# CESNET/GPUJPEG

Measured on NVIDIA H100. Metric: Mpix/s encode+decode 8k RGB q75, higher is better.
Workload: dtype f32+i32 (u8 in, i16 coefficients)

## Files before the change

### gpujpeg_b200/csrc/gj_dct.cu

```cuda
#include <cuda_runtime.h>
#include <stdint.h>
#include <stdlib.h>
#include <string.h>

#include <tuple>
#include <type_traits>

#include "gj_device.cuh"
#include "gj_internal.h"
#include "gj_launch.cuh"

namespace {

constexpr int TB = 64;
constexpr int NT = 192;
constexpr int STRIP_PX = TB * 8;
constexpr int GROUPS = 8 * (STRIP_PX / 4);
constexpr int BLK_F = 68;
constexpr int K1_SMEM = 3 * TB * BLK_F * 4;
constexpr int K1_OUT_STRIDE = 9;
constexpr int K4_PLANE = 8 * STRIP_PX;

struct FdctParams {
    float fwd_zz[2][64];
};
struct IdctParams {
    uint16_t q_zz[GJ_MAX_COMP][64];
};

__device__ __forceinline__ uint32_t pack4_sat_u8(int p0, int p1, int p2, int p3)
{
    uint32_t hi, d;
    asm("cvt.pack.sat.u8.s32.b32 %0, %1, %2, %3;" : "=r"(hi) : "r"(p3), "r"(p2), "r"(0));
    asm("cvt.pack.sat.u8.s32.b32 %0, %1, %2, %3;" : "=r"(d) : "r"(p1), "r"(p0), "r"(hi));
    return d;
}

__device__ __forceinline__ uint64_t quantise_pack(const float (&v)[64], const float* __restrict__ tab, uint32_t (&packed)[32])
{
    uint32_t mlo = 0, mhi = 0;
#pragma unroll
    for ( int k = 0; k < 64; k += 2 ) {
        const uint32_t b0 = gj_quant_bits(v[gj_zz2nat(k)], tab[k]);
        const uint32_t b1 = gj_quant_bits(v[gj_zz2nat(k + 1)], tab[k + 1]);
        packed[k >> 1] = __byte_perm(b0, b1, 0x5410);
        if ( k < 32 ) {
            if ( b0 != GJ_QUANT_ZERO ) mlo |= 1u << (k & 31);
            if ( b1 != GJ_QUANT_ZERO ) mlo |= 1u << ((k + 1) & 31);
        }
        else {
            if ( b0 != GJ_QUANT_ZERO ) mhi |= 1u << (k & 31);
            if ( b1 != GJ_QUANT_ZERO ) mhi |= 1u << ((k + 1) & 31);
        }
    }
    return (uint64_t)mhi << 32 | mlo;
}
__device__ __forceinline__ void quantise_store(const float (&v)[64], const float* __restrict__ tab, int16_t* __restrict__ coef_blk,
                                               uint64_t* __restrict__ nz)
{
    uint32_t packed[32];
    *nz = quantise_pack(v, tab, packed);
    uint4* dst = reinterpret_cast<uint4*>(coef_blk);
#pragma unroll
    for ( int i = 0; i < 8; i++ )
        dst[i] = make_uint4(packed[4 * i], packed[4 * i + 1], packed[4 * i + 2], packed[4 * i + 3]);
}


template <int VEC>
__global__ void __launch_bounds__(NT)
k_fdct_rgb444(const uint8_t* __restrict__ raw, int width, int height, size_t pitch, int16_t* __restrict__ coef,
              uint64_t* __restrict__ nzmask, int bcx, int nblk, const __grid_constant__ FdctParams prm)
{
    gj_pdl_wait();
    extern __shared__ __align__(16) uint8_t smem[];
    float* s_pl = reinterpret_cast<float*>(smem);

    const int bx0 = blockIdx.x * TB;
    const int by = blockIdx.y;
    const int x0 = bx0 * 8;
    const int vw = min(STRIP_PX, width - x0);
    const int vh = min(8, height - by * 8);
    const uint8_t* src = raw + (size_t)by * 8 * pitch + (size_t)x0 * 3;

    constexpr int ITERS = (GROUPS + NT - 1) / NT;
    uint32_t w0[ITERS], w1[ITERS], w2[ITERS];
#pragma unroll
    for ( int it = 0; it < ITERS; it++ ) {
        const int g = threadIdx.x + it * NT;
        const int row = g >> 7, gx = g & 127, px0 = gx * 4;
        w0[it] = w1[it] = w2[it] = 0u;
        if ( g < GROUPS && row < vh && px0 < vw ) {
            const uint8_t* p = src + (size_t)row * pitch + gx * 12;
            if ( VEC == 4 && px0 + 4 <= vw ) {
                const uint32_t* w = reinterpret_cast<const uint32_t*>(p);
                w0[it] = __ldg(w);
                w1[it] = __ldg(w + 1);
                w2[it] = __ldg(w + 2);
            }
            else {
                const int nb = min(12, (vw - px0) * 3);
                uint32_t b[12];
#pragma unroll
                for ( int i = 0; i < 12; i++ )
                    b[i] = i < nb ? (uint32_t)__ldg(p + i) : 0u;
                w0[it] = b[0] | b[1] << 8 | b[2] << 16 | b[3] << 24;
                w1[it] = b[4] | b[5] << 8 | b[6] << 16 | b[7] << 24;
                w2[it] = b[8] | b[9] << 8 | b[10] << 16 | b[11] << 24;
            }
        }
    }
#pragma unroll
    for ( int it = 0; it < ITERS; it++ ) {
        const int g = threadIdx.x + it * NT;
        if ( g >= GROUPS ) break;
        const int row = g >> 7, gx = g & 127, px0 = gx * 4;
        float4 y4 = make_float4(0.f, 0.f, 0.f, 0.f), cb4 = y4, cr4 = y4;
        if ( row < vh && px0 < vw ) {
            const uint32_t a0 = w0[it], a1 = w1[it], a2 = w2[it];
            gj_rgb_to_ycbcr_m(gj_byte_as_magic(a0, 0), gj_byte_as_magic(a0, 1), gj_byte_as_magic(a0, 2), y4.x, cb4.x, cr4.x);
            gj_rgb_to_ycbcr_m(gj_byte_as_magic(a0, 3), gj_byte_as_magic(a1, 0), gj_byte_as_magic(a1, 1), y4.y, cb4.y, cr4.y);
            gj_rgb_to_ycbcr_m(gj_byte_as_magic(a1, 2), gj_byte_as_magic(a1, 3), gj_byte_as_magic(a2, 0), y4.z, cb4.z, cr4.z);
            gj_rgb_to_ycbcr_m(gj_byte_as_magic(a2, 1), gj_byte_as_magic(a2, 2), gj_byte_as_magic(a2, 3), y4.w, cb4.w, cr4.w);
            if ( px0 + 4 > vw ) {
                if ( px0 + 1 >= vw ) { y4.y = cb4.y = cr4.y = 0.f; }
                if ( px0 + 2 >= vw ) { y4.z = cb4.z = cr4.z = 0.f; }
                if ( px0 + 3 >= vw ) { y4.w = cb4.w = cr4.w = 0.f; }
            }
        }
        const int off = (gx >> 1) * BLK_F + row * 8 + (gx & 1) * 4;
        *reinterpret_cast<float4*>(s_pl + off) = y4;
        *reinterpret_cast<float4*>(s_pl + TB * BLK_F + off) = cb4;
        *reinterpret_cast<float4*>(s_pl + 2 * TB * BLK_F + off) = cr4;
    }
    __syncthreads();

    const int comp = threadIdx.x >> 6;
    const int b = threadIdx.x & 63;
    const bool active = bx0 + b < bcx;
    float v[64];
    {
        const float4* in = reinterpret_cast<const float4*>(s_pl + (comp * TB + b) * BLK_F);
#pragma unroll
        for ( int i = 0; i < 16; i++ ) {
            const float4 t = in[i];
            v[4 * i] = t.x; v[4 * i + 1] = t.y; v[4 * i + 2] = t.z; v[4 * i + 3] = t.w;
        }
    }
    __syncthreads();
    gj_fdct_block(v);
    uint4* const s_out = reinterpret_cast<uint4*>(smem);
    {
        uint32_t packed[32];
        const uint64_t nz = quantise_pack(v, prm.fwd_zz[comp == 0 ? 0 : 1], packed);
        const size_t bi = (size_t)comp * nblk + (size_t)by * bcx + bx0 + b;
        if ( active ) nzmask[bi] = nz;
#pragma unroll
        for ( int i = 0; i < 8; i++ )
            s_out[threadIdx.x * K1_OUT_STRIDE + i] = make_uint4(packed[4 * i], packed[4 * i + 1], packed[4 * i + 2], packed[4 * i + 3]);
    }
    __syncthreads();
#pragma unroll
    for ( int k = 0; k < 8; k++ ) {
        const int q = threadIdx.x + k * NT;
        const int slot = q >> 3, part = q & 7;
        const int c2 = slot >> 6, b2 = slot & 63;
        if ( bx0 + b2 < bcx ) {
            const size_t bi = (size_t)c2 * nblk + (size_t)by * bcx + bx0 + b2;
            reinterpret_cast<uint4*>(coef + bi * 64)[part] = s_out[slot * K1_OUT_STRIDE + part];
        }
    }
}

constexpr int K1T_RAW = 8 * STRIP_PX * 3;
constexpr int K1T_SMEM = K1_SMEM + K1T_RAW + 16;

__device__ __forceinline__ uint32_t smem_u32(const void* p) { return (uint32_t)__cvta_generic_to_shared(p); }
__device__ __forceinline__ void mbar_init(uint32_t bar, uint32_t count)
{
    asm volatile("mbarrier.init.shared::cta.b64 [%0], %1;" ::"r"(bar), "r"(count));
}
__device__ __forceinline__ void mbar_expect_tx(uint32_t bar, uint32_t bytes)
{
    asm volatile("mbarrier.arrive.expect_tx.shared::cta.b64 _, [%0], %1;" ::"r"(bar), "r"(bytes) : "memory");
}
__device__ __forceinline__ void mbar_wait(uint32_t bar, uint32_t parity)
{
    asm volatile(
        "{\n"
        ".reg .pred p;\n"
        "WAIT_%=:\n"
        "mbarrier.try_wait.parity.shared::cta.b64 p, [%0], %1;\n"
        "@p bra DONE_%=;\n"
        "bra WAIT_%=;\n"
        "DONE_%=:\n"
        "}\n" ::"r"(bar),
        "r"(parity)
        : "memory");
}
__device__ __forceinline__ void bulk_g2s(uint32_t dst, const void* src, uint32_t bytes, uint32_t bar)
{
    asm volatile("cp.async.bulk.shared::cluster.global.mbarrier::complete_tx::bytes [%0], [%1], %2, [%3];" ::"r"(dst), "l"(src),
// ... 53 lines not shown
            *reinterpret_cast<float4*>(s_pl + off) = y4;
            *reinterpret_cast<float4*>(s_pl + TB * BLK_F + off) = cb4;
            *reinterpret_cast<float4*>(s_pl + 2 * TB * BLK_F + off) = cr4;
        }
        __syncthreads();
        if ( threadIdx.x == 0 && strip + (int)gridDim.x < n_strips ) {
            asm volatile("fence.proxy.async.shared::cta;" ::: "memory");
            request(strip + gridDim.x);
        }

        const int comp = threadIdx.x >> 6;
        const int b = threadIdx.x & 63;
        if ( bx0 + b < bcx ) {
            float v[64];
            const float4* in = reinterpret_cast<const float4*>(s_pl + (comp * TB + b) * BLK_F);
#pragma unroll
            for ( int i = 0; i < 16; i++ ) {
                const float4 t = in[i];
                v[4 * i] = t.x; v[4 * i + 1] = t.y; v[4 * i + 2] = t.z; v[4 * i + 3] = t.w;
            }
            gj_fdct_block(v);
            const size_t bi = (size_t)comp * nblk + (size_t)by * bcx + bx0 + b;
            quantise_store(v, prm.fwd_zz[comp == 0 ? 0 : 1], coef + bi * 64, nzmask + bi);
        }
        __syncthreads();
    }
}

struct SsGrid {
    int bcx[3], bcy[3], blk_off[3];
};

template <int HS, int VS, int VEC>
__global__ void __launch_bounds__(TB * VS + 2 * TB / HS)
k_fdct_rgb_ss(const uint8_t* __restrict__ raw, int width, int height, size_t pitch, int16_t* __restrict__ coef,
              uint64_t* __restrict__ nzmask, const __grid_constant__ SsGrid grid, const __grid_constant__ FdctParams prm)
{
    gj_pdl_wait();
    constexpr int NTS = TB * VS + 2 * TB / HS;
    constexpr int CB = TB / HS;
    constexpr int ITERS = (GROUPS + NTS - 1) / NTS;
    extern __shared__ __align__(16) uint8_t smem[];
    float* s_y = reinterpret_cast<float*>(smem);
    float* s_c = s_y + VS * TB * BLK_F;

    const int bx0 = blockIdx.x * TB;
    const int x0 = bx0 * 8;
    const int y0 = blockIdx.y * 8 * VS;
    const int vw = min(STRIP_PX, width - x0);
    const uint8_t* src = raw + (size_t)y0 * pitch + (size_t)x0 * 3;

#pragma unroll
    for ( int half = 0; half < VS; half++ ) {
        const int vh = min(8, height - y0 - half * 8);
        uint32_t w0[ITERS], w1[ITERS], w2[ITERS];
#pragma unroll
        for ( int it = 0; it < ITERS; it++ ) {
            const int g = threadIdx.x + it * NTS;
            const int row = g >> 7, gx = g & 127, px0 = gx * 4;
            w0[it] = w1[it] = w2[it] = 0u;
            if ( g < GROUPS && row < vh && px0 < vw ) {
                const uint8_t* p = src + (size_t)(half * 8 + row) * pitch + gx * 12;
                if ( VEC == 4 && px0 + 4 <= vw ) {
                    const uint32_t* w = reinterpret_cast<const uint32_t*>(p);
                    w0[it] = __ldg(w);
                    w1[it] = __ldg(w + 1);
                    w2[it] = __ldg(w + 2);
                }
                else {
                    const int nb = min(12, (vw - px0) * 3);
                    uint32_t b[12];
#pragma unroll
                    for ( int i = 0; i < 12; i++ )
                        b[i] = i < nb ? (uint32_t)__ldg(p + i) : 0u;
                    w0[it] = b[0] | b[1] << 8 | b[2] << 16 | b[3] << 24;
                    w1[it] = b[4] | b[5] << 8 | b[6] << 16 | b[7] << 24;
                    w2[it] = b[8] | b[9] << 8 | b[10] << 16 | b[11] << 24;
                }
            }
        }
#pragma unroll
        for ( int it = 0; it < ITERS; it++ ) {
            const int g = threadIdx.x + it * NTS;
            if ( g >= GROUPS ) break;
            const int row = g >> 7, gx = g & 127, px0 = gx * 4;
            float4 y4 = make_float4(0.f, 0.f, 0.f, 0.f), cb4 = y4, cr4 = y4;
            if ( row < vh && px0 < vw ) {
                const uint32_t a0 = w0[it], a1 = w1[it], a2 = w2[it];
                gj_rgb_to_ycbcr_m(gj_byte_as_magic(a0, 0), gj_byte_as_magic(a0, 1), gj_byte_as_magic(a0, 2), y4.x, cb4.x, cr4.x);
                gj_rgb_to_ycbcr_m(gj_byte_as_magic(a0, 3), gj_byte_as_magic(a1, 0), gj_byte_as_magic(a1, 1), y4.y, cb4.y, cr4.y);
                gj_rgb_to_ycbcr_m(gj_byte_as_magic(a1, 2), gj_byte_as_magic(a1, 3), gj_byte_as_magic(a2, 0), y4.z, cb4.z, cr4.z);
                gj_rgb_to_ycbcr_m(gj_byte_as_magic(a2, 1), gj_byte_as_magic(a2, 2), gj_byte_as_magic(a2, 3), y4.w, cb4.w, cr4.w);
                if ( px0 + 4 > vw ) {
                    if ( px0 + 1 >= vw ) { y4.y = cb4.y = cr4.y = 0.f; }
                    if ( px0 + 2 >= vw ) { y4.z = cb4.z = cr4.z = 0.f; }
                    if ( px0 + 3 >= vw ) { y4.w = cb4.w = cr4.w = 0.f; }
                }
            }
            *reinterpret_cast<float4*>(s_y + (half * TB + (gx >> 1)) * BLK_F + row * 8 + (gx & 1) * 4) = y4;
            const int srow = half * 8 + row;
            if ( VS == 1 || (srow & 1) == 0 ) {
                const int crow = srow / VS;
                if ( HS == 1 ) {
                    const int off = (gx >> 1) * BLK_F + crow * 8 + (gx & 1) * 4;
                    *reinterpret_cast<float4*>(s_c + off) = cb4;
                    *reinterpret_cast<float4*>(s_c + CB * BLK_F + off) = cr4;
                }
                else {
                    const int off = (gx >> 2) * BLK_F + crow * 8 + (gx & 3) * 2;
                    *reinterpret_cast<float2*>(s_c + off) = make_float2(cb4.x, cb4.z);
                    *reinterpret_cast<float2*>(s_c + CB * BLK_F + off) = make_float2(cr4.x, cr4.z);
                }
            }
        }
    }
    __syncthreads();

    auto locate = [&](int t, int& comp, int& bx, int& by) {
        if ( t < TB * VS ) {
            comp = 0;
            bx = bx0 + (t & (TB - 1));
            by = blockIdx.y * VS + t / TB;
        }
        else {
            const int u = t - TB * VS;
            comp = 1 + u / CB;
            bx = bx0 / HS + u % CB;
            by = blockIdx.y;
        }
        return bx < grid.bcx[comp] && by < grid.bcy[comp];
    };
    int comp, bx, by;
    const bool active = locate(threadIdx.x, comp, bx, by);
    float v[64];
    {
        const float4* in = reinterpret_cast<const float4*>(s_y + threadIdx.x * BLK_F);
#pragma unroll
        for ( int i = 0; i < 16; i++ ) {
            const float4 t = in[i];
            v[4 * i] = t.x; v[4 * i + 1] = t.y; v[4 * i + 2] = t.z; v[4 * i + 3] = t.w;
        }
    }
    __syncthreads();
    gj_fdct_block(v);
    uint4* const s_out = reinterpret_cast<uint4*>(smem);
    {
        uint32_t packed[32];
        const uint64_t nz = quantise_pack(v, prm.fwd_zz[comp == 0 ? 0 : 1], packed);
        if ( active ) nzmask[(size_t)grid.blk_off[comp] + (size_t)by * grid.bcx[comp] + bx] = nz;
#pragma unroll
        for ( int i = 0; i < 8; i++ )
            s_out[threadIdx.x * K1_OUT_STRIDE + i] = make_uint4(packed[4 * i], packed[4 * i + 1], packed[4 * i + 2], packed[4 * i + 3]);
    }
    __syncthreads();
#pragma unroll
    for ( int k = 0; k < 8; k++ ) {
        const int q = threadIdx.x + k * NTS;
        const int slot = q >> 3, part = q & 7;
        int c2, bx2, by2;
        if ( locate(slot, c2, bx2, by2) ) {
            const size_t bi = (size_t)grid.blk_off[c2] + (size_t)by2 * grid.bcx[c2] + bx2;
            reinterpret_cast<uint4*>(coef + bi * 64)[part] = s_out[slot * K1_OUT_STRIDE + part];
        }
    }
}

struct LjGrid {
    int bcx[3], bcy[3], blk_off[3];
    int wib[3], hib[3];
};
struct LjParams {
    uint32_t recip[2][64];
    uint16_t q[2][64];
};

template <int HS, int VS, int NC>
struct LjShape {
    static constexpr int NTS = TB * VS + (NC == 3 ? 2 * TB / HS : 0);
    static constexpr int CB = TB / HS;
    static constexpr int PLANE = 8 * VS * STRIP_PX;
    static constexpr int OUT = NTS * K1_OUT_STRIDE * 16;
    static constexpr int SMEM = (NC * PLANE > OUT ? NC * PLANE : OUT) + NTS * 4;
};

template <int N>
__device__ __forceinline__ void lj_row(const uint8_t* __restrict__ row, int x, int vw, int (&out)[N])
{
    if ( x + N <= vw ) {
        const uint32_t* w = reinterpret_cast<const uint32_t*>(row + x);
#pragma unroll
        for ( int i = 0; i < N / 4; i++ ) {
            const uint32_t v = w[i];
#pragma unroll
            for ( int j = 0; j < 4; j++ )
                out[4 * i + j] = (int)((v >> (8 * j)) & 255u);
// ... 1208 lines not shown
```

### gpujpeg_b200/csrc/gj_decoder.c

```c
#include <stdlib.h>
#include <string.h>

#include "gj_internal.h"

#define GJ_MK_OTHER_CAP 256
#define GJ_CTA_BYTES0 (64 * 1024)
#define GJ_MK_WORDS (8 + 4 * GJ_MK_OTHER_CAP)

#define GJ_STRIPES 8
#define GJ_STRIPE_MIN_BYTES ((size_t)8 << 20)

struct gpujpeg_decoder {
    gj_stream_t stream;
    gj_stream_t copy_stream;
    void* ev_stripe[GJ_STRIPES]; void* ev_done;
    int stripes;
    size_t stripe_min_bytes;
    int k3_parts;
    int device;
    int verbose, perf_stats;
    struct gpujpeg_parameters param;
    struct gpujpeg_image_parameters param_image;
    struct gj_geometry geo;
    int initialised;
// ... 1547 lines not shown

GPUJPEG_API int gpujpegx_decoder_subsequence_rounds(struct gpujpeg_decoder* d)
{
    if ( !d || !d->last_valid || !d->used_subsequences ) return -1;
    return gj_subseq_rounds(d->d_ss_scratch, d->stream);
}

GPUJPEG_API int gpujpegx_decoder_run_resident(struct gpujpeg_decoder* d, uint8_t* d_out, int stage_mask)
{
    if ( !d || !d->last_valid ) return -1;
    if ( d->last_progressive ) {
        static const int comp_tq[GJ_MAX_COMP] = {0, 1, 2, 3};
        if ( (stage_mask & 4) &&
             gj_launch_marker_scan(d->d_file, d->last_ecs_begin, d->last_args.file_size, d->d_cta, d->d_list_pos, d->d_list_code,
                                   d->d_list_cpos, d->last_list_cap, d->d_clean, d->d_mk, d->d_mk + 8, GJ_MK_OTHER_CAP, d->stream) )
            return -1;
        if ( (stage_mask & 1) && gj_launch_progressive_decode(&d->last_prog, d->stream) ) return -1;
        if ( (stage_mask & 2) && launch_k4(d, comp_tq, d_out ? d_out : d->d_raw, 0, d->k4.mcu_rows) ) return -1;
        return 0;
    }
    if ( (stage_mask & 4) && !d->used_segment_info &&
         gj_launch_marker_scan(d->d_file, d->last_ecs_begin, d->last_args.file_size, d->d_cta, d->d_list_pos, d->d_list_code,
                               d->d_list_cpos, d->last_list_cap, d->d_clean, d->d_mk, d->d_mk + 8, GJ_MK_OTHER_CAP, d->stream) )
        return -1;
    if ( (stage_mask & 1) && d->crop && gj_cuda_memset_async(d->d_cext, 0, d->geo.coef_count / 64, d->stream) ) return -1;
    if ( (stage_mask & 1) && gj_launch_huffman_decode(&d->last_args, d->stream) ) return -1;
    if ( (stage_mask & 2) && launch_k4(d, d->last_tq, d_out ? d_out : d->d_raw, 0, d->k4.mcu_rows) ) return -1;
    return 0;
}

GPUJPEG_API int gpujpegx_decoder_get_coefficients(struct gpujpeg_decoder* d, int16_t* out, size_t count)
{
    if ( !d || !d->initialised || !d->last_valid || count != d->geo.coef_count ) return -1;
    if ( gj_coef_to_host_natural(d->d_coef, d->d_cext, count, out, d->stream) ) return -1;
    return d->k4.dequantize;
}
```

### gpujpeg_b200/csrc/gj_device.cuh

```cuda
#ifndef GJ_DEVICE_CUH
#define GJ_DEVICE_CUH

#include <stdint.h>
#include <math.h>

#include "gj_internal.h"

#if defined(__CUDA_ARCH__)
#define GJ_HD __host__ __device__ __forceinline__
#define GJ_FADD(a, b) __fadd_rn((a), (b))
#define GJ_FSUB(a, b) __fsub_rn((a), (b))
#define GJ_FMUL(a, b) __fmul_rn((a), (b))
#define GJ_FMA(a, b, c) __fmaf_rn((a), (b), (c))
#define GJ_RINT(a) __float2int_rn(a)
#elif defined(__CUDACC__)
#define GJ_HD __host__ __device__ __forceinline__
#define GJ_FADD(a, b) ((a) + (b))
#define GJ_FSUB(a, b) ((a) - (b))
#define GJ_FMUL(a, b) ((a) * (b))
#define GJ_FMA(a, b, c) fmaf((a), (b), (c))
#define GJ_RINT(a) ((int)rintf(a))
#else
#define GJ_HD static inline
#define GJ_FADD(a, b) ((a) + (b))
// ... 1 lines not shown
#define GJ_FMUL(a, b) ((a) * (b))
#define GJ_FMA(a, b, c) fmaf((a), (b), (c))
#define GJ_RINT(a) ((int)rintf(a))
#endif


GJ_HD constexpr int gj_zz2nat(int k)
{
    constexpr int t[64] = {0,  1,  8,  16, 9,  2,  3,  10, 17, 24, 32, 25, 18, 11, 4,  5,  12, 19, 26, 33, 40, 48,
                           41, 34, 27, 20, 13, 6,  7,  14, 21, 28, 35, 42, 49, 56, 57, 50, 43, 36, 29, 22, 15, 23,
                           30, 37, 44, 51, 58, 59, 52, 45, 38, 31, 39, 46, 53, 60, 61, 54, 47, 55, 62, 63};
    return t[k];
}
GJ_HD constexpr int gj_nat2zz(int n)
{
    constexpr int t[64] = {0,  1,  5,  6,  14, 15, 27, 28, 2,  4,  7,  13, 16, 26, 29, 42, 3,  8,  12, 17, 25, 30,
                           41, 43, 9,  11, 18, 24, 31, 40, 44, 53, 10, 19, 23, 32, 39, 45, 52, 54, 20, 22, 33, 38,
                           46, 51, 55, 60, 21, 34, 37, 47, 50, 56, 59, 61, 35, 36, 48, 49, 57, 58, 62, 63};
    return t[n];
}

GJ_HD int gj_coef_src(int k, int transpose, int neg_x, int neg_y, int* negate)
{
    const int n = gj_zz2nat(k), v = n >> 3, u = n & 7;
    const int sv = transpose ? u : v, su = transpose ? v : u;
    *negate = ((neg_x & su) ^ (neg_y & sv)) & 1;
    return gj_nat2zz(sv * 8 + su);
}


GJ_HD int gj_cext_of(int last_zz) { return (last_zz >> 3) + 1; }
GJ_HD bool gj_cext_holds(int ext, int k) { return (k >> 3) < ext; }

#if defined(__CUDACC__)
__device__ __forceinline__ void gj_load_coef_block(const int16_t* __restrict__ blk, int ext, uint32_t (&packed)[32])
{
    const uint4* src = reinterpret_cast<const uint4*>(blk);
#pragma unroll
    for ( int i = 0; i < 8; i++ ) {
        const uint4 t = i < ext ? __ldg(src + i) : make_uint4(0u, 0u, 0u, 0u);
        packed[4 * i] = t.x; packed[4 * i + 1] = t.y; packed[4 * i + 2] = t.z; packed[4 * i + 3] = t.w;
    }
}
#endif


#define GJ_MAGIC23 8388608.0f
#define GJ_MAGIC15 12582912.0f
GJ_HD float gj_byte_as_magic(uint32_t word, int i)
{
#if defined(__CUDA_ARCH__)
    return __uint_as_float(__byte_perm(word, 0x4B000000u, 0x7440 + i));
#else
    union { uint32_t u; float f; } c;
    c.u = 0x4B000000u | ((word >> (8 * i)) & 0xFFu);
    return c.f;
#endif
}
GJ_HD float gj_scale255_m(float cm) { return fmaxf(cm, fmaf(cm, 2.0f, -(GJ_MAGIC23 + 254.0f))) - GJ_MAGIC23; }
GJ_HD float gj_round_clamp255(float acc) { return fminf(acc + GJ_MAGIC15, GJ_MAGIC15 + 255.0f) - GJ_MAGIC15; }
GJ_HD void gj_rgb_to_ycbcr_m(float rm, float gm, float bm, float& y, float& cb, float& cr)
{
    const float r = gj_scale255_m(rm), g = gj_scale255_m(gm), b = gj_scale255_m(bm);
    const float e = 1.0f / 512.0f;
    y = gj_round_clamp255(fmaf(77.0f / 256.0f, r, fmaf(150.0f / 256.0f, g, fmaf(29.0f / 256.0f, b, e))));
    cb = gj_round_clamp255(fmaf(-43.0f / 256.0f, r, fmaf(-85.0f / 256.0f, g, fmaf(128.0f / 256.0f, b, 128.0f + e))));
    cr = gj_round_clamp255(fmaf(128.0f / 256.0f, r, fmaf(-107.0f / 256.0f, g, fmaf(-21.0f / 256.0f, b, 128.0f + e))));
}
GJ_HD void gj_rgb_to_ycbcr(float r, float g, float b, float& y, float& cb, float& cr)
{
    gj_rgb_to_ycbcr_m(r + GJ_MAGIC23, g + GJ_MAGIC23, b + GJ_MAGIC23, y, cb, cr);
}

GJ_HD int gj_clamp8(int v) { return v < 0 ? 0 : (v > 255 ? 255 : v); }
GJ_HD void gj_ycbcr_to_rgb_raw(int Y, int Cb, int Cr, int& r, int& g, int& b)
{
    const int y = Y * 256 + ((Y + 1) & 0x100) + 128;
    const int cb = Cb - 128, cr = Cr - 128;
    r = (y + 359 * cr) >> 8;
    g = (y - 88 * cb - 183 * cr) >> 8;
    b = (y + 454 * cb) >> 8;
}
GJ_HD void gj_ycbcr_to_rgb(int Y, int Cb, int Cr, int& r, int& g, int& b)
{
    gj_ycbcr_to_rgb_raw(Y, Cb, Cr, r, g, b);
    r = gj_clamp8(r);
    g = gj_clamp8(g);
    b = gj_clamp8(b);
}


GJ_HD void gj_fdct1(float& a0, float& a1, float& a2, float& a3, float& a4, float& a5, float& a6, float& a7,
                    const float shift)
{
    const float d0 = GJ_FADD(a0, a7), d1 = GJ_FADD(a1, a6), d2 = GJ_FADD(a2, a5), d3 = GJ_FADD(a3, a4);
    const float d4 = GJ_FSUB(a3, a4), d5 = GJ_FSUB(a2, a5), d6 = GJ_FSUB(a1, a6), d7 = GJ_FSUB(a0, a7);
    const float e0 = GJ_FADD(d0, d3), e1 = GJ_FADD(d1, d2), e2 = GJ_FSUB(d1, d2), e3 = GJ_FSUB(d0, d3);
    const float ed = GJ_FADD(e2, e3);
    const float o0 = GJ_FADD(d4, d5), o1 = GJ_FADD(d5, d6), o2 = GJ_FADD(d6, d7);
    const float od5 = GJ_FMUL(GJ_FSUB(o0, o2), 0.382683433f);
    const float od4 = GJ_FMA(1.306562965f, o2, od5);
    const float od3 = GJ_FMA(-0.707106781f, o1, d7);
    const float od2 = GJ_FMA(0.541196100f, o0, od5);
    const float od1 = GJ_FMA(0.707106781f, o1, d7);
// ... 911 lines not shown
```

### gpujpeg_b200/csrc/gj_encoder.c

```c
#include <assert.h>
#include <stdlib.h>
#include <string.h>

#include "gj_internal.h"

#define GJ_STRIPES 8
#define GJ_STRIPE_MIN_BYTES ((size_t)8 << 20)

struct gpujpeg_encoder {
    gj_stream_t stream;
    int device;
    struct gpujpeg_parameters param;
    struct gpujpeg_image_parameters param_image;
    int initialised;
    struct gj_geometry geo;
    int input_mode;
    uint8_t* d_planes; size_t d_planes_size;
    struct gj_raw_layout raw;
    int quality;
    enum gpujpeg_header_type header_type;
    enum gpujpeg_header_type header_written;
    int flipped;
    int flip_mode;
    unsigned channel_remap;
// ... 1137 lines not shown
    if ( (stage_mask & 1) && launch_k1(e, d_raw) ) return -1;
    if ( (stage_mask & 8) && launch_stats(e) ) return -1;
    if ( (stage_mask & 2) && launch_k2(e) ) return -1;
    return 0;
}

GPUJPEG_API int gpujpegx_encoder_get_symbol_counts(struct gpujpeg_encoder* e, uint64_t out[2][2][256])
{
    if ( !e || !e->initialised || !e->counts_valid || !out ) return -1;
    if ( gj_cuda_memcpy_d2h_async(e->h_counts, e->d_counts, GJ_HUFF_COUNTS_BYTES, e->stream) || gj_cuda_stream_sync(e->stream) )
        return -1;
    memcpy(out, e->h_counts, GJ_HUFF_COUNTS_BYTES);
    return 0;
}

GPUJPEG_API long long gpujpegx_encoder_get_stream(struct gpujpeg_encoder* e, uint8_t* out, size_t capacity)
{
    if ( !e || !e->initialised || e->with_segment_info || !e->d_info_cur ) return -1;
    if ( gj_cuda_memcpy_d2h_async(e->h_info, e->d_info_cur, 32, e->stream) || gj_cuda_stream_sync(e->stream) ) return -1;
    const size_t total = (size_t)e->h_info[0];
    if ( e->h_info[1] || total < e->header_size + 2 || total > e->d_stream_size ) return -1;
    if ( !out ) return (long long)total;
    if ( total > capacity ) return -1;
    if ( gj_cuda_memcpy_d2h_async(out + e->header_size, e->d_stream + e->header_size, total - e->header_size, e->stream) ||
         gj_cuda_stream_sync(e->stream) )
        return -1;
    memcpy(out, e->header, e->header_size);
    return (long long)total;
}

GPUJPEG_API int gpujpegx_encoder_get_coefficients(struct gpujpeg_encoder* e, int16_t* out, size_t count)
{
    if ( !e || !e->initialised || count != e->geo.coef_count ) return -1;
    return gj_coef_to_host_natural(e->d_coef, NULL, count, out, e->stream);
}
```

### gpujpeg_b200/csrc/gj_huffman.cu

```cuda
#include <cuda_runtime.h>
#include <stdint.h>

#include "gj_device.cuh"
#include "gj_internal.h"
#include "gj_launch.cuh"

namespace {

constexpr unsigned FULL = 0xFFFFFFFFu;

__device__ __forceinline__ int warp_incl_scan(int v, int lane)
{
#pragma unroll
    for ( int d = 1; d < 32; d <<= 1 ) {
        const int t = __shfl_up_sync(FULL, v, d);
        if ( lane >= d ) v += t;
    }
    return v;
}

__device__ __forceinline__ int scan_of_segment(const gj_scan_layout& L, int g)
{
    return (g >= L.scan_seg_begin[1]) + (g >= L.scan_seg_begin[2]) + (g >= L.scan_seg_begin[3]);
}
// ... 1293 lines not shown
            uint4* dst = reinterpret_cast<uint4*>(s_cmp);
            for ( uint32_t i = lane; i < (need + 3u) >> 2; i += 32 )
                dst[i] = __ldg(src + i);
        }
        __syncwarp();
        const uint32_t* w = staged ? s_cmp + ((cs >> 2) - wbase) : a.d_clean + (cs >> 2);
        CleanSource c;
        c.n = 0;
        if ( live ) src_init(c, w, w + ((ce >> 2) - (cs >> 2)) + 4, (cs & 3u) * 8u);
        decode_blocks(c);
    }
    else {
        BitSource r;
        r.n = 0;
        if ( live ) src_init(r, file + start, file_end);
        decode_blocks(r);
    }
}

__global__ void __launch_bounds__(256) k_rst_check(const __grid_constant__ gj_huff_dec_args a)
{
    gj_pdl_wait();
    const int g = blockIdx.x * 256 + threadIdx.x;
    if ( g >= a.seg_count ) return;
    const int scan = scan_of_segment(a.lay, g);
    const int s = g - a.lay.scan_seg_begin[scan];
    if ( s > 0 && a.d_list_code[a.first_rank[scan] + (uint32_t)s - 1u] != (uint8_t)(0xD0 + ((s - 1) & 7)) ) atomicExch(a.d_error, 1u);
}

__constant__ uint8_t c_zz2nat[64] = {
    0,  1,  8,  16, 9,  2,  3,  10, 17, 24, 32, 25, 18, 11, 4,  5,  12, 19, 26, 33, 40, 48,
    41, 34, 27, 20, 13, 6,  7,  14, 21, 28, 35, 42, 49, 56, 57, 50, 43, 36, 29, 22, 15, 23,
    30, 37, 44, 51, 58, 59, 52, 45, 38, 31, 39, 46, 53, 60, 61, 54, 47, 55, 62, 63};
__global__ void k_coef_to_natural(const int16_t* __restrict__ in, const uint8_t* __restrict__ cext, int16_t* __restrict__ out,
                                  size_t nblocks)
{
    const size_t i = (size_t)blockIdx.x * blockDim.x + threadIdx.x;
    if ( i >= nblocks * 64 ) return;
    const int k = (int)(i & 63);
    out[(i & ~(size_t)63) + c_zz2nat[k]] = !cext || gj_cext_holds(cext[i >> 6], k) ? in[i] : (int16_t)0;
}

}

static unsigned long long* place_status_of(const struct gj_huff_enc_args* a) { return reinterpret_cast<unsigned long long*>(a->d_seg_off); }

extern "C" int gj_huffman_encode_parts_eligible(const struct gj_huff_enc_args* a)
{
    return a->lay.simple && a->seg_mcu * a->lay.bpm <= HP_MAXBLK;
}

extern "C" int gj_launch_huffman_encode_part(const struct gj_huff_enc_args* a, int first, const int lo[GJ_MAX_COMP],
                                             const int n[GJ_MAX_COMP], gj_stream_t stream)
{
    const int seg_count = a->lay.scan_seg_begin[GJ_MAX_COMP];
    if ( a->seg_mcu * a->lay.bpm > HP_MAXBLK ) return -1;
    if ( first && !a->info_is_zero && cudaMemsetAsync(a->d_info, 0, 32, stream) != cudaSuccess ) return -1;
    SegPick pick;
    pick.total = 0;
    pick.zero_status = first;
    for ( int k = 0; k < GJ_MAX_COMP; k++ ) {
        const bool real = k < a->lay.scan_count;
        pick.n[k] = real ? n[k] : 0;
        pick.lo[k] = real ? a->lay.scan_seg_begin[k] + lo[k] : 0;
        if ( pick.n[k] < 0 || (real && (lo[k] < 0 || pick.lo[k] + pick.n[k] > a->lay.scan_seg_begin[k + 1])) ) return -1;
        pick.total += pick.n[k];
    }
    if ( pick.total == 0 && !first ) return 0;
    const int n_status = (seg_count + CP_SEGS - 1) / CP_SEGS;
    static int attr_done_p[64];
    int dev = 0;
    if ( cudaGetDevice(&dev) != cudaSuccess || dev < 0 || dev >= 64 ) return -1;
    if ( !__atomic_load_n(&attr_done_p[dev], __ATOMIC_ACQUIRE) ) {
// ... 157 lines not shown
        const int cmp_max = (int)(HD_THREADS / 32 * HD_CMP_MAX + 64);
        if ( cudaFuncSetAttribute(k_huff_decode<true, true, false>, cudaFuncAttributeMaxDynamicSharedMemorySize, cmp_max) != cudaSuccess ||
             cudaFuncSetAttribute(k_huff_decode<false, true, false>, cudaFuncAttributeMaxDynamicSharedMemorySize, cmp_max) != cudaSuccess ||
             cudaFuncSetAttribute(k_huff_decode<true, true, true>, cudaFuncAttributeMaxDynamicSharedMemorySize, cmp_max) != cudaSuccess ||
             cudaFuncSetAttribute(k_huff_decode<false, true, true>, cudaFuncAttributeMaxDynamicSharedMemorySize, cmp_max) != cudaSuccess )
            return -1;
        __atomic_store_n(&attr_done[dev], 1, __ATOMIC_RELEASE);
    }
    auto launch = [&](auto kernel) {
        gj_launch_pdl(kernel, dim3(grid), dim3(HD_THREADS), smem, stream, a->d_file, a->d_file + a->file_size, a->d_seg_off,
                      owners, a->seg_mcu, *a, own, a->d_coef, a->d_cext, a->d_tables);
    };
    if ( pick ) {
        if ( own.cmp_words ) {
            if ( a->dequantize ) launch(k_huff_decode<true, true, true>);
            else launch(k_huff_decode<false, true, true>);
        }
        else {
            if ( a->dequantize ) launch(k_huff_decode<true, false, true>);
            else launch(k_huff_decode<false, false, true>);
        }
    }
    else if ( own.cmp_words ) {
        if ( a->dequantize ) launch(k_huff_decode<true, true, false>);
        else launch(k_huff_decode<false, true, false>);
    }
    else {
        if ( a->dequantize ) launch(k_huff_decode<true, false, false>);
        else launch(k_huff_decode<false, false, false>);
    }
    return cudaGetLastError() == cudaSuccess ? 0 : -1;
}

extern "C" int gj_coef_to_host_natural(const int16_t* d_coef, const uint8_t* d_cext, size_t count, int16_t* h_out, gj_stream_t stream)
{
    int16_t* d_tmp = nullptr;
    if ( cudaMalloc(&d_tmp, count * sizeof(int16_t)) != cudaSuccess ) return -1;
    const size_t nblocks = count / 64;
    k_coef_to_natural<<<(unsigned)((count + 255) / 256), 256, 0, stream>>>(d_coef, d_cext, d_tmp, nblocks);
    cudaMemcpyAsync(h_out, d_tmp, count * sizeof(int16_t), cudaMemcpyDeviceToHost, stream);
    const cudaError_t e = cudaStreamSynchronize(stream);
    cudaFree(d_tmp);
    return e == cudaSuccess ? 0 : -1;
}
```

### gpujpeg_b200/csrc/gj_internal.h

```cpp
#ifndef GJ_INTERNAL_H
#define GJ_INTERNAL_H

#include <stddef.h>
#include <stdint.h>
#include <stdio.h>

#include "../../include/gpujpeg_b200.h"

#ifdef __cplusplus
extern "C" {
#endif

#define GJ_MAX_COMP 4
#define GJ_SOS_LEN_1 10

#define GJ_ERR(...) (void)(fprintf(stderr, "[GPUJPEG] [Error] " __VA_ARGS__))
#define GJ_WARN(...) (void)(fprintf(stderr, "[GPUJPEG] [Warning] " __VA_ARGS__))
#define GJ_VERBOSE(v, ...) do { if ( (v) >= GPUJPEG_LL_VERBOSE ) (void)fprintf(stderr, "[GPUJPEG] [Verbose] " __VA_ARGS__); } while ( 0 )
#define GJ_DEBUG(v, ...) do { if ( (v) >= GPUJPEG_LL_DEBUG ) (void)fprintf(stderr, "[GPUJPEG] [Debug] " __VA_ARGS__); } while ( 0 )

extern const uint8_t gj_zigzag_to_natural[64];
extern const uint8_t gj_natural_to_zigzag[64];

struct gj_huff_spec {
// ... 456 lines not shown
    const uint8_t* d_cext;
    int src_blk_off[GJ_MAX_COMP];
    int16_t* d_dst;
    uint64_t* d_nzmask;
    int dst_blk_off[GJ_MAX_COMP];
    int comp_count;
    int dst_blocks;
    int transpose, neg_x, neg_y;
    struct gj_blk_map blk[GJ_MAX_COMP];
    uint32_t* d_range;
};
int gj_launch_coef_transform(const struct gj_coef_transform_args* a, gj_stream_t stream);

struct gj_coef_frame {
    const struct gj_geometry* geo;
    const int16_t* d_coef;
    const uint8_t* d_cext;
    int progressive;
    enum gpujpeg_color_space color_space;
    uint8_t qt[GJ_MAX_COMP][64];
    int tq[GJ_MAX_COMP];
    struct gpujpeg_image_metadata metadata;
    const uint8_t* com;
    size_t com_size;
};
int gj_decoder_decode_coefficients(struct gpujpeg_decoder* d, const uint8_t* image, size_t image_size, struct gj_coef_frame* f);

int gj_encoder_setup_coefficients(struct gpujpeg_encoder* e, const struct gpujpeg_parameters* p, int width, int height,
                                  const uint8_t comp_q[GJ_MAX_COMP][64], const uint8_t comp_tq[GJ_MAX_COMP], const uint8_t* com,
                                  size_t com_size, const struct gpujpeg_image_metadata* metadata, int16_t** d_coef,
                                  uint64_t** d_nzmask, const struct gj_geometry** geo);
int gj_encoder_finish(struct gpujpeg_encoder* e, uint8_t** out, size_t* out_size);

int gj_coef_to_host_natural(const int16_t* d_coef, const uint8_t* d_cext, size_t count, int16_t* h_out, gj_stream_t stream);

int gj_cuda_malloc(void** p, size_t size);
int gj_cuda_free(void* p);
int gj_cuda_malloc_host(void** p, size_t size);
int gj_cuda_free_host(void* p);
int gj_cuda_memcpy_h2d_async(void* dst, const void* src, size_t size, gj_stream_t s);
int gj_cuda_memcpy_d2h_async(void* dst, const void* src, size_t size, gj_stream_t s);
int gj_cuda_memcpy_d2d_async(void* dst, const void* src, size_t size, gj_stream_t s);
int gj_cuda_memset_async(void* dst, int v, size_t size, gj_stream_t s);
int gj_cuda_stream_sync(gj_stream_t s);
int gj_cuda_stream_create(gj_stream_t* s);
int gj_cuda_event_create(void** ev);
void gj_cuda_event_destroy(void* ev);
int gj_cuda_event_record(void* ev, gj_stream_t s);
int gj_cuda_stream_wait_event(gj_stream_t s, void* ev);
void gj_cuda_stream_destroy(gj_stream_t s);
int gj_cuda_enable_peer(int peer);
int gj_cuda_memcpy_peer_async(void* dst, int dst_dev, const void* src, int src_dev, size_t size, gj_stream_t s);
int gj_cuda_pointer_is_device(const void* p);
const char* gj_cuda_last_error(void);
struct gj_timer { void* start; void* stop; int armed; };
int gj_timer_create(struct gj_timer* t);
void gj_timer_destroy(struct gj_timer* t);
void gj_timer_start(struct gj_timer* t, gj_stream_t s);
void gj_timer_stop(struct gj_timer* t, gj_stream_t s);
double gj_timer_ms(struct gj_timer* t);
int gj_cuda_device_count(void);
int gj_cuda_sm_count(void);
int gj_cuda_device_props(int dev, struct gpujpeg_device_info* info);
int gj_cuda_set_device(int dev);
int gj_cuda_get_device(void);
void gj_cuda_device_reset(void);

// ... 5 lines not shown
```

Measured before the change: 58620.

## Store only live coefficient chunks and use dp4a integer color conversion

The forward DCT kernels now write only the 16-byte coefficient chunks up to the last nonzero zigzag position, as derived from the nonzero mask, and skip the trailing zero chunks. The goal is to cut global write traffic. Consumers must then treat the unwritten chunks as zero, so the coefficient export masks them using nzmask. The RGB to YCbCr step is replaced by an integer dp4a/byte-permute version, which may change rounding. The subsampled kernel also gets a minimum-blocks-per-SM launch bound.

After: 60670 (median of 6 runs). +3.5%, better.

```diff
diff --git a/gpujpeg_b200/csrc/gj_dct.cu b/gpujpeg_b200/csrc/gj_dct.cu
--- a/gpujpeg_b200/csrc/gj_dct.cu
+++ b/gpujpeg_b200/csrc/gj_dct.cu
@@ -19,6 +19,7 @@
 constexpr int BLK_F = 68;
 constexpr int K1_SMEM = 3 * TB * BLK_F * 4;
 constexpr int K1_OUT_STRIDE = 9;
+constexpr int k1_ctas_per_sm(int nt) { return 228 * 1024 / (nt * BLK_F * 4 + 1024); }
 constexpr int K4_PLANE = 8 * STRIP_PX;
 
 struct FdctParams {
@@ -64,6 +65,39 @@
 #pragma unroll
     for ( int i = 0; i < 8; i++ )
         dst[i] = make_uint4(packed[4 * i], packed[4 * i + 1], packed[4 * i + 2], packed[4 * i + 3]);
+}
+
+__device__ __forceinline__ void ycc4_clipped(uint32_t w0, uint32_t w1, uint32_t w2, int left, float4& y4, float4& cb4, float4& cr4)
+{
+    float y[4], cb[4], cr[4];
+    gj_rgb4_to_ycbcr(w0, w1, w2, y, cb, cr);
+    y4 = make_float4(y[0], y[1], y[2], y[3]);
+    cb4 = make_float4(cb[0], cb[1], cb[2], cb[3]);
+    cr4 = make_float4(cr[0], cr[1], cr[2], cr[3]);
+    if ( left < 4 ) {
+        if ( left <= 1 ) { y4.y = cb4.y = cr4.y = 0.f; }
+        if ( left <= 2 ) { y4.z = cb4.z = cr4.z = 0.f; }
+        if ( left <= 3 ) { y4.w = cb4.w = cr4.w = 0.f; }
+    }
+}
+
+__device__ __forceinline__ void stage_live_block(uint4* s_out, uint8_t* s_live, int slot, uint64_t nz, const uint32_t (&packed)[32])
+{
+    const int live = (gj_coef_live_chunks(nz) + 1) & ~1;
+    s_live[slot] = (uint8_t)live;
+#pragma unroll
+    for ( int i = 0; i < 8; i++ )
+        if ( i < live ) s_out[slot * K1_OUT_STRIDE + i] = make_uint4(packed[4 * i], packed[4 * i + 1], packed[4 * i + 2], packed[4 * i + 3]);
+}
+
+__device__ __forceinline__ void load_staged(const uint4* s_out, const uint8_t* s_live, int nt, uint4 (&chunk)[8], int (&live)[8])
+{
+#pragma unroll
+    for ( int k = 0; k < 8; k++ ) {
+        const int q = threadIdx.x + k * nt;
+        chunk[k] = s_out[(q >> 3) * K1_OUT_STRIDE + (q & 7)];
+        live[k] = s_live[q >> 3];
+    }
 }
 
 
@@ -116,18 +150,8 @@
         if ( g >= GROUPS ) break;
         const int row = g >> 7, gx = g & 127, px0 = gx * 4;
         float4 y4 = make_float4(0.f, 0.f, 0.f, 0.f), cb4 = y4, cr4 = y4;
-        if ( row < vh && px0 < vw ) {
-            const uint32_t a0 = w0[it], a1 = w1[it], a2 = w2[it];
-            gj_rgb_to_ycbcr_m(gj_byte_as_magic(a0, 0), gj_byte_as_magic(a0, 1), gj_byte_as_magic(a0, 2), y4.x, cb4.x, cr4.x);
-            gj_rgb_to_ycbcr_m(gj_byte_as_magic(a0, 3), gj_byte_as_magic(a1, 0), gj_byte_as_magic(a1, 1), y4.y, cb4.y, cr4.y);
-            gj_rgb_to_ycbcr_m(gj_byte_as_magic(a1, 2), gj_byte_as_magic(a1, 3), gj_byte_as_magic(a2, 0), y4.z, cb4.z, cr4.z);
-            gj_rgb_to_ycbcr_m(gj_byte_as_magic(a2, 1), gj_byte_as_magic(a2, 2), gj_byte_as_magic(a2, 3), y4.w, cb4.w, cr4.w);
-            if ( px0 + 4 > vw ) {
-                if ( px0 + 1 >= vw ) { y4.y = cb4.y = cr4.y = 0.f; }
-                if ( px0 + 2 >= vw ) { y4.z = cb4.z = cr4.z = 0.f; }
-                if ( px0 + 3 >= vw ) { y4.w = cb4.w = cr4.w = 0.f; }
-            }
-        }
+        if ( row < vh && px0 < vw )
+            ycc4_clipped(w0[it], w1[it], w2[it], vw - px0, y4, cb4, cr4);
         const int off = (gx >> 1) * BLK_F + row * 8 + (gx & 1) * 4;
         *reinterpret_cast<float4*>(s_pl + off) = y4;
         *reinterpret_cast<float4*>(s_pl + TB * BLK_F + off) = cb4;
@@ -150,24 +174,27 @@
     __syncthreads();
     gj_fdct_block(v);
     uint4* const s_out = reinterpret_cast<uint4*>(smem);
+    uint8_t* const s_live = smem + NT * K1_OUT_STRIDE * 16;
+    static_assert(NT * (K1_OUT_STRIDE * 16 + 1) <= K1_SMEM, "output staging must fit into the planar staging area");
     {
         uint32_t packed[32];
         const uint64_t nz = quantise_pack(v, prm.fwd_zz[comp == 0 ? 0 : 1], packed);
         const size_t bi = (size_t)comp * nblk + (size_t)by * bcx + bx0 + b;
         if ( active ) nzmask[bi] = nz;
-#pragma unroll
-        for ( int i = 0; i < 8; i++ )
-            s_out[threadIdx.x * K1_OUT_STRIDE + i] = make_uint4(packed[4 * i], packed[4 * i + 1], packed[4 * i + 2], packed[4 * i + 3]);
+        stage_live_block(s_out, s_live, threadIdx.x, nz, packed);
     }
     __syncthreads();
+    uint4 chunk[8];
+    int live[8];
+    load_staged(s_out, s_live, NT, chunk, live);
 #pragma unroll
     for ( int k = 0; k < 8; k++ ) {
         const int q = threadIdx.x + k * NT;
         const int slot = q >> 3, part = q & 7;
         const int c2 = slot >> 6, b2 = slot & 63;
-        if ( bx0 + b2 < bcx ) {
+        if ( bx0 + b2 < bcx && part < live[k] ) {
             const size_t bi = (size_t)c2 * nblk + (size_t)by * bcx + bx0 + b2;
-            reinterpret_cast<uint4*>(coef + bi * 64)[part] = s_out[slot * K1_OUT_STRIDE + part];
+            reinterpret_cast<uint4*>(coef + bi * 64)[part] = chunk[k];
         }
     }
 }
@@ -287,7 +314,7 @@
 };
 
 template <int HS, int VS, int VEC>
-__global__ void __launch_bounds__(TB * VS + 2 * TB / HS)
+__global__ void __launch_bounds__(TB * VS + 2 * TB / HS, k1_ctas_per_sm(TB * VS + 2 * TB / HS))
 k_fdct_rgb_ss(const uint8_t* __restrict__ raw, int width, int height, size_t pitch, int16_t* __restrict__ coef,
               uint64_t* __restrict__ nzmask, const __grid_constant__ SsGrid grid, const __grid_constant__ FdctParams prm)
 {
@@ -340,18 +367,8 @@
             if ( g >= GROUPS ) break;
             const int row = g >> 7, gx = g & 127, px0 = gx * 4;
             float4 y4 = make_float4(0.f, 0.f, 0.f, 0.f), cb4 = y4, cr4 = y4;
-            if ( row < vh && px0 < vw ) {
-                const uint32_t a0 = w0[it], a1 = w1[it], a2 = w2[it];
-                gj_rgb_to_ycbcr_m(gj_byte_as_magic(a0, 0), gj_byte_as_magic(a0, 1), gj_byte_as_magic(a0, 2), y4.x, cb4.x, cr4.x);
-                gj_rgb_to_ycbcr_m(gj_byte_as_magic(a0, 3), gj_byte_as_magic(a1, 0), gj_byte_as_magic(a1, 1), y4.y, cb4.y, cr4.y);
-                gj_rgb_to_ycbcr_m(gj_byte_as_magic(a1, 2), gj_byte_as_magic(a1, 3), gj_byte_as_magic(a2, 0), y4.z, cb4.z, cr4.z);
-                gj_rgb_to_ycbcr_m(gj_byte_as_magic(a2, 1), gj_byte_as_magic(a2, 2), gj_byte_as_magic(a2, 3), y4.w, cb4.w, cr4.w);
-                if ( px0 + 4 > vw ) {
-                    if ( px0 + 1 >= vw ) { y4.y = cb4.y = cr4.y = 0.f; }
-                    if ( px0 + 2 >= vw ) { y4.z = cb4.z = cr4.z = 0.f; }
-                    if ( px0 + 3 >= vw ) { y4.w = cb4.w = cr4.w = 0.f; }
-                }
-            }
+            if ( row < vh && px0 < vw )
+                ycc4_clipped(w0[it], w1[it], w2[it], vw - px0, y4, cb4, cr4);
             *reinterpret_cast<float4*>(s_y + (half * TB + (gx >> 1)) * BLK_F + row * 8 + (gx & 1) * 4) = y4;
             const int srow = half * 8 + row;
             if ( VS == 1 || (srow & 1) == 0 ) {
@@ -399,23 +416,26 @@
     __syncthreads();
     gj_fdct_block(v);
     uint4* const s_out = reinterpret_cast<uint4*>(smem);
+    uint8_t* const s_live = smem + NTS * K1_OUT_STRIDE * 16;
+    static_assert(BLK_F * 4 >= K1_OUT_STRIDE * 16 + 1, "output staging must fit into the planar staging area (NTS blocks)");
     {
         uint32_t packed[32];
         const uint64_t nz = quantise_pack(v, prm.fwd_zz[comp == 0 ? 0 : 1], packed);
         if ( active ) nzmask[(size_t)grid.blk_off[comp] + (size_t)by * grid.bcx[comp] + bx] = nz;
-#pragma unroll
-        for ( int i = 0; i < 8; i++ )
-            s_out[threadIdx.x * K1_OUT_STRIDE + i] = make_uint4(packed[4 * i], packed[4 * i + 1], packed[4 * i + 2], packed[4 * i + 3]);
+        stage_live_block(s_out, s_live, threadIdx.x, nz, packed);
     }
     __syncthreads();
+    uint4 chunk[8];
+    int live[8];
+    load_staged(s_out, s_live, NTS, chunk, live);
 #pragma unroll
     for ( int k = 0; k < 8; k++ ) {
         const int q = threadIdx.x + k * NTS;
         const int slot = q >> 3, part = q & 7;
         int c2, bx2, by2;
-        if ( locate(slot, c2, bx2, by2) ) {
+        if ( part < live[k] && locate(slot, c2, bx2, by2) ) {
             const size_t bi = (size_t)grid.blk_off[c2] + (size_t)by2 * grid.bcx[c2] + bx2;
-            reinterpret_cast<uint4*>(coef + bi * 64)[part] = s_out[slot * K1_OUT_STRIDE + part];
+            reinterpret_cast<uint4*>(coef + bi * 64)[part] = chunk[k];
         }
     }
 }
diff --git a/gpujpeg_b200/csrc/gj_decoder.c b/gpujpeg_b200/csrc/gj_decoder.c
--- a/gpujpeg_b200/csrc/gj_decoder.c
+++ b/gpujpeg_b200/csrc/gj_decoder.c
@@ -1603,6 +1603,6 @@
 GPUJPEG_API int gpujpegx_decoder_get_coefficients(struct gpujpeg_decoder* d, int16_t* out, size_t count)
 {
     if ( !d || !d->initialised || !d->last_valid || count != d->geo.coef_count ) return -1;
-    if ( gj_coef_to_host_natural(d->d_coef, d->d_cext, count, out, d->stream) ) return -1;
+    if ( gj_coef_to_host_natural(d->d_coef, d->d_cext, NULL, count, out, d->stream) ) return -1;
     return d->k4.dequantize;
 }
diff --git a/gpujpeg_b200/csrc/gj_device.cuh b/gpujpeg_b200/csrc/gj_device.cuh
--- a/gpujpeg_b200/csrc/gj_device.cuh
+++ b/gpujpeg_b200/csrc/gj_device.cuh
@@ -57,6 +57,18 @@
 GJ_HD int gj_cext_of(int last_zz) { return (last_zz >> 3) + 1; }
 GJ_HD bool gj_cext_holds(int ext, int k) { return (k >> 3) < ext; }
 
+GJ_HD int gj_coef_live_chunks(uint64_t nz)
+{
+#if defined(__CUDA_ARCH__)
+    const int last = 63 - __clzll((long long)nz);
+#else
+    int last = -1;
+    for ( int k = 0; k < 64; k++ )
+        if ( (nz >> k) & 1u ) last = k;
+#endif
+    return last < 16 ? 2 : (last >> 3) + 1;
+}
+
 #if defined(__CUDACC__)
 __device__ __forceinline__ void gj_load_coef_block(const int16_t* __restrict__ blk, int ext, uint32_t (&packed)[32])
 {
@@ -95,6 +107,75 @@
 GJ_HD void gj_rgb_to_ycbcr(float r, float g, float b, float& y, float& cb, float& cr)
 {
     gj_rgb_to_ycbcr_m(r + GJ_MAGIC23, g + GJ_MAGIC23, b + GJ_MAGIC23, y, cb, cr);
+}
+
+GJ_HD uint32_t gj_prmt(uint32_t a, uint32_t b, uint32_t sel)
+{
+#if defined(__CUDA_ARCH__)
+    return __byte_perm(a, b, sel);
+#else
+    const uint64_t x = (uint64_t)b << 32 | a;
+    uint32_t d = 0;
+    for ( int i = 0; i < 4; i++ )
+        d |= (uint32_t)((x >> (8 * ((sel >> (4 * i)) & 7u))) & 0xFFu) << (8 * i);
+    return d;
+#endif
+}
+GJ_HD int gj_dp4a_uu(uint32_t a, uint32_t b, int c)
+{
+#if defined(__CUDA_ARCH__)
+    int d;
+    asm("dp4a.u32.u32 %0, %1, %2, %3;" : "=r"(d) : "r"(a), "r"(b), "r"(c));
+    return d;
+#else
+    for ( int i = 0; i < 4; i++ )
+        c += (int)((a >> (8 * i)) & 0xFFu) * (int)((b >> (8 * i)) & 0xFFu);
+    return c;
+#endif
+}
+GJ_HD int gj_dp4a_us(uint32_t a, uint32_t b, int c)
+{
+#if defined(__CUDA_ARCH__)
+    int d;
+    asm("dp4a.u32.s32 %0, %1, %2, %3;" : "=r"(d) : "r"(a), "r"(b), "r"(c));
+    return d;
+#else
+    for ( int i = 0; i < 4; i++ )
+        c += (int)((a >> (8 * i)) & 0xFFu) * (int)(int8_t)((b >> (8 * i)) & 0xFFu);
+    return c;
+#endif
+}
+GJ_HD float gj_bits_float(uint32_t u)
+{
+#if defined(__CUDA_ARCH__)
+    return __uint_as_float(u);
+#else
+    union { uint32_t u; float f; } c;
+    c.u = u;
+    return c.f;
+#endif
+}
+GJ_HD uint32_t gj_eq255_4(uint32_t w) { return (((w & 0x7F7F7F7Fu) + 0x01010101u) & w & 0x80808080u) >> 7; }
+template <int at>
+GJ_HD void gj_ycc_int_px(uint32_t p, uint32_t m, float& y, float& cb, float& cr)
+{
+    constexpr uint32_t KY = (77u | 150u << 8 | 29u << 16) << (8 * at);
+    constexpr uint32_t KCB = (43u | 85u << 8 | 0x80u << 16) << (8 * at);
+    constexpr uint32_t KCR = (0x80u | 107u << 8 | 21u << 16) << (8 * at);
+    const int sy = gj_dp4a_uu(m, KY, gj_dp4a_uu(p, KY, 128));
+    const int tb = gj_dp4a_us(m, KCB, gj_dp4a_us(p, KCB, -32897));
+    const int tr = gj_dp4a_us(m, KCR, gj_dp4a_us(p, KCR, -32897));
+    y = fminf(gj_bits_float((uint32_t)(sy >> 8) + 0x4B000000u), GJ_MAGIC23 + 255.0f) - GJ_MAGIC23;
+    cb = (GJ_MAGIC23 + 511.0f) - fmaxf(gj_bits_float((uint32_t)((tb >> 8) + 0x4B000200)), GJ_MAGIC23 + 256.0f);
+    cr = (GJ_MAGIC23 + 511.0f) - fmaxf(gj_bits_float((uint32_t)((tr >> 8) + 0x4B000200)), GJ_MAGIC23 + 256.0f);
+}
+GJ_HD void gj_rgb4_to_ycbcr(uint32_t w0, uint32_t w1, uint32_t w2, float (&y)[4], float (&cb)[4], float (&cr)[4])
+{
+    const uint32_t m0 = gj_eq255_4(w0), m1 = gj_eq255_4(w1), m2 = gj_eq255_4(w2);
+    gj_ycc_int_px<0>(w0, m0, y[0], cb[0], cr[0]);
+    gj_ycc_int_px<0>(gj_prmt(w0, w1, 0x6543), gj_prmt(m0, m1, 0x6543), y[1], cb[1], cr[1]);
+    gj_ycc_int_px<0>(gj_prmt(w1, w2, 0x5432), gj_prmt(m1, m2, 0x5432), y[2], cb[2], cr[2]);
+    gj_ycc_int_px<1>(w2, m2, y[3], cb[3], cr[3]);
 }
 
 GJ_HD int gj_clamp8(int v) { return v < 0 ? 0 : (v > 255 ? 255 : v); }
diff --git a/gpujpeg_b200/csrc/gj_encoder.c b/gpujpeg_b200/csrc/gj_encoder.c
--- a/gpujpeg_b200/csrc/gj_encoder.c
+++ b/gpujpeg_b200/csrc/gj_encoder.c
@@ -1193,5 +1193,5 @@
 GPUJPEG_API int gpujpegx_encoder_get_coefficients(struct gpujpeg_encoder* e, int16_t* out, size_t count)
 {
     if ( !e || !e->initialised || count != e->geo.coef_count ) return -1;
-    return gj_coef_to_host_natural(e->d_coef, NULL, count, out, e->stream);
-}
+    return gj_coef_to_host_natural(e->d_coef, NULL, e->d_nzmask, count, out, e->stream);
+}
diff --git a/gpujpeg_b200/csrc/gj_huffman.cu b/gpujpeg_b200/csrc/gj_huffman.cu
--- a/gpujpeg_b200/csrc/gj_huffman.cu
+++ b/gpujpeg_b200/csrc/gj_huffman.cu
@@ -1349,13 +1349,14 @@
     0,  1,  8,  16, 9,  2,  3,  10, 17, 24, 32, 25, 18, 11, 4,  5,  12, 19, 26, 33, 40, 48,
     41, 34, 27, 20, 13, 6,  7,  14, 21, 28, 35, 42, 49, 56, 57, 50, 43, 36, 29, 22, 15, 23,
     30, 37, 44, 51, 58, 59, 52, 45, 38, 31, 39, 46, 53, 60, 61, 54, 47, 55, 62, 63};
-__global__ void k_coef_to_natural(const int16_t* __restrict__ in, const uint8_t* __restrict__ cext, int16_t* __restrict__ out,
-                                  size_t nblocks)
+__global__ void k_coef_to_natural(const int16_t* __restrict__ in, const uint8_t* __restrict__ cext,
+                                  const uint64_t* __restrict__ nzmask, int16_t* __restrict__ out, size_t nblocks)
 {
     const size_t i = (size_t)blockIdx.x * blockDim.x + threadIdx.x;
     if ( i >= nblocks * 64 ) return;
     const int k = (int)(i & 63);
-    out[(i & ~(size_t)63) + c_zz2nat[k]] = !cext || gj_cext_holds(cext[i >> 6], k) ? in[i] : (int16_t)0;
+    const bool held = cext ? gj_cext_holds(cext[i >> 6], k) : nzmask ? (k >> 3) < gj_coef_live_chunks(nzmask[i >> 6]) : true;
+    out[(i & ~(size_t)63) + c_zz2nat[k]] = held ? in[i] : (int16_t)0;
 }
 
 }
@@ -1579,12 +1580,13 @@
     return cudaGetLastError() == cudaSuccess ? 0 : -1;
 }
 
-extern "C" int gj_coef_to_host_natural(const int16_t* d_coef, const uint8_t* d_cext, size_t count, int16_t* h_out, gj_stream_t stream)
+extern "C" int gj_coef_to_host_natural(const int16_t* d_coef, const uint8_t* d_cext, const uint64_t* d_nzmask, size_t count,
+                                       int16_t* h_out, gj_stream_t stream)
 {
     int16_t* d_tmp = nullptr;
     if ( cudaMalloc(&d_tmp, count * sizeof(int16_t)) != cudaSuccess ) return -1;
     const size_t nblocks = count / 64;
-    k_coef_to_natural<<<(unsigned)((count + 255) / 256), 256, 0, stream>>>(d_coef, d_cext, d_tmp, nblocks);
+    k_coef_to_natural<<<(unsigned)((count + 255) / 256), 256, 0, stream>>>(d_coef, d_cext, d_nzmask, d_tmp, nblocks);
     cudaMemcpyAsync(h_out, d_tmp, count * sizeof(int16_t), cudaMemcpyDeviceToHost, stream);
     const cudaError_t e = cudaStreamSynchronize(stream);
     cudaFree(d_tmp);
diff --git a/gpujpeg_b200/csrc/gj_internal.h b/gpujpeg_b200/csrc/gj_internal.h
--- a/gpujpeg_b200/csrc/gj_internal.h
+++ b/gpujpeg_b200/csrc/gj_internal.h
@@ -512,7 +512,8 @@
                                   uint64_t** d_nzmask, const struct gj_geometry** geo);
 int gj_encoder_finish(struct gpujpeg_encoder* e, uint8_t** out, size_t* out_size);
 
-int gj_coef_to_host_natural(const int16_t* d_coef, const uint8_t* d_cext, size_t count, int16_t* h_out, gj_stream_t stream);
+int gj_coef_to_host_natural(const int16_t* d_coef, const uint8_t* d_cext, const uint64_t* d_nzmask, size_t count, int16_t* h_out,
+                            gj_stream_t stream);
 
 int gj_cuda_malloc(void** p, size_t size);
 int gj_cuda_free(void* p);
diff --git a/profiles/k1_live.py b/profiles/k1_live.py
--- /dev/null
+++ b/profiles/k1_live.py
@@ -0,0 +1,84 @@
+import argparse
+import json
+import os
+import subprocess
+import sys
+
+HERE = os.path.dirname(os.path.abspath(__file__))
+W, H = 7680, 4320
+CASES = [("photo", "4:4:4", 0, 36), ("random", "4:4:4", 0, 36), ("photo", "4:2:0", 1, 6)]
+
+
+def worker(root, launches):
+    sys.path[:0] = [root, os.path.join(root, "tests")]
+    import numpy as np
+    import torch
+    import _oracle as o
+    import gpujpeg_b200 as g
+    dev = torch.device("cuda", 0)
+    stream = torch.cuda.current_stream().cuda_stream
+
+    def median_us(fn):
+        for _ in range(10):
+            fn()
+        ev = [(torch.cuda.Event(enable_timing=True), torch.cuda.Event(enable_timing=True)) for _ in range(launches)]
+        for e0, e1 in ev:
+            e0.record()
+            fn()
+            e1.record()
+        torch.cuda.synchronize()
+        return float(np.median([e0.elapsed_time(e1) * 1e3 for e0, e1 in ev]))
+
+    out = {"tree": root}
+    for kind, ss, il, rst in CASES:
+        img = o.gen_image(kind, W, H)
+        d_raw = torch.from_numpy(img).to(dev)
+        enc = g.Encoder(stream=stream, pinned_output=True)
+        enc.encode(d_raw, 75, rst, il, subsampling=ss)
+        name = "%s_%s" % (kind, ss.replace(":", ""))
+        out["k1_us_" + name] = round(median_us(lambda: enc.run_resident(d_raw, 1)), 2)
+        out["k2_us_" + name] = round(median_us(lambda: enc.run_resident(d_raw, 2)), 2)
+        enc.close()
+    print(json.dumps(out), flush=True)
+
+
+def count():
+    sys.path.insert(0, os.path.join(os.path.dirname(HERE), "tests"))
+    import numpy as np
+    import _oracle as o
+    img = o.gen_image("photo", W, H)
+    _, coef = o.encode(img, 75, 36, 0, want_coef=True, threads=os.cpu_count() or 4)
+    zz = coef.reshape(-1, 64)[:, o.ZIGZAG]
+    nz = zz != 0
+    last = np.where(nz.any(axis=1), 63 - np.argmax(nz[:, ::-1], axis=1), -1)
+    chunks = np.maximum(2, last // 8 + 1)
+    per_comp = chunks.reshape(3, -1)
+    res = {"blocks": int(chunks.size), "whole_blocks_MB": round(chunks.size * 128 / 1e6, 1),
+           "live_MB": round(int(chunks.sum()) * 16 / 1e6, 1),
+           "chunks_per_block": [round(float(c.mean()), 3) for c in per_comp]}
+    print(json.dumps(res))
+
+
+def main():
+    ap = argparse.ArgumentParser()
+    ap.add_argument("--trees", nargs="*", default=[])
+    ap.add_argument("--rounds", type=int, default=3)
+    ap.add_argument("--launches", type=int, default=60)
+    ap.add_argument("--worker", default=None)
+    ap.add_argument("--count", action="store_true")
+    a = ap.parse_args()
+    if a.count:
+        return count()
+    if a.worker:
+        return worker(a.worker, a.launches)
+    q = subprocess.run(["nvidia-smi", "--query-gpu=name,power.limit,clocks.max.sm", "--format=csv,noheader"],
+                       capture_output=True, text=True)
+    print(json.dumps({"gpu": q.stdout.strip()}), flush=True)
+    for _ in range(a.rounds):
+        for t in a.trees:
+            subprocess.run([sys.executable, os.path.abspath(__file__), "--worker", os.path.abspath(t), "--launches",
+                            str(a.launches)], check=True)
+
+
+if __name__ == "__main__":
+    main()
```
